# sandialabs/PyNucleus

Hardware: AMD Instinct MI355X
Metric: element-pairs/sec assembled (2D P1 fractional s=0.5, dense) + % fp64 roofline (higher is better)
Workload: dtype f64; 1 GPU; 2D unit disc (uniform_disc refined 7x, 98304 cells), P1, 48769 DoFs, fractional s=0.5, horizon=inf, dense getDense incl. zeroExterior; 4831887360 element pairs/step; noRef=7, num_dofs=48769, num_cells=98304, parallelism=block rows of the upper triangle dealt over 1 GPU(s), row-owned one-sided slabs

## Files before the change

include/pnl_hip.h:

```cpp
#ifndef PNL_HIP_H
#define PNL_HIP_H
#include <stdint.h>

#ifdef __cplusplus
extern "C" {
#endif

typedef struct pnl_context pnl_context;

enum pnl_status {
    PNL_OK = 0,
    PNL_ERR_INVALID = -1,
    PNL_ERR_UNSUPPORTED = -2,
    PNL_ERR_HIP = -3,
    PNL_ERR_STATE = -4,
    PNL_ERR_ORDER = -5
};

enum pnl_kernel_type { PNL_FRACTIONAL = 0, PNL_INDICATOR = 1, PNL_PERIDYNAMIC = 2, PNL_GAUSSIAN = 3, PNL_EXPONENTIAL = 4,
                       PNL_GAUSSIAN_BOUNDARY = 5, PNL_EXPONENTIAL_BOUNDARY = 6 };

typedef struct {
    int32_t ktype;
    int32_t interaction;
// ... 133 lines not shown

int pnl_set_order_function(pnl_context *ctx, const pnl_order_function *f, const double *cell_smax, const double *facet_smax,
                           double c0, double bc0, double sing_fac, double bsing_fac);
int pnl_set_order_vertex_values(pnl_context *ctx, int nv, const double *values_host);
int pnl_upload_pointwise_rules(pnl_context *ctx, int which, int panel, int nkeys, int M, int rows, const double *nodes,
                               const double *w, const double *phi0, const double *phi1);
int pnl_assemble_dense_pointwise(pnl_context *ctx, double *A, int64_t ldA, int zero_exterior, int cell_begin, int cell_end,
                                 int npairs, const int32_t *pairs, int nbpairs, const int32_t *bpairs);
int pnl_assemble_pairs_masked_pointwise(pnl_context *ctx, int np, const int32_t *pairs, const uint64_t *masks, const int32_t *rule,
                                        double *data);
int pnl_assemble_boundary_masked_pointwise(pnl_context *ctx, int ni, const int32_t *cells, const int32_t *facets, const uint32_t *masks,
                                           const int32_t *rule, const double *sv, double fac, double *data, double *diag);

int pnl_get_counters(pnl_context *ctx, int64_t *out, int n);
int pnl_get_phase_ms(pnl_context *ctx, float *out, int n);
int pnl_get_settled_tiles(pnl_context *ctx, int32_t *tiles, int64_t ntiles);
int pnl_get_settled_lists(pnl_context *ctx, uint16_t *codes, uint16_t *lists, int64_t ntiles);
int pnl_uniform_lane_layout(int nc, const int32_t *cells, const int32_t *dofs, int mode, int nthreads, int32_t *sizes, uint8_t *lane_cell,
                            int16_t *lds_col, int8_t *vorder, int16_t *cell_col, double *mult, double *seconds);
enum pnl_kernel_slot { PNL_K_TILE_GENERAL = 0, PNL_K_TILE_UNIFORM2, PNL_K_TILE_UNIFORM3, PNL_K_TILE_UNIFORM4, PNL_K_FOLD_MIRROR,
                       PNL_K_WORKLIST, PNL_K_TILE_SETTLED, PNL_NUM_KERNEL_SLOTS };
int pnl_get_kernel_ms(pnl_context *ctx, float *out, int n);

typedef struct pnl_tree pnl_tree;
typedef struct pnl_nfplan pnl_nfplan;
int pnl_tree_build(int N, int dim, const double *boxes, const int64_t *d2c_ptr, const int32_t *d2c_idx, int nc, double eta,
                   int min_size, int max_levels, int do_admissibility, pnl_tree **out);
int pnl_tree_build_blocks(int N, int dim, const double *boxes, const int64_t *d2c_ptr, const int32_t *d2c_idx, int nc, double eta,
                          int min_size, int max_levels, int do_admissibility, const int32_t *dof_block, int mixed_block,
                          pnl_tree **out);
// ... 174 lines not shown
```

pynucleus_amd/_lib.py:

```python
import ctypes as C
import os
import numpy as np

_HERE = os.path.dirname(os.path.abspath(__file__))
LIB_PATH = os.environ.get('PNL_LIB', os.path.join(_HERE, 'libpnl_hip.so'))

PNL_OK = 0
PNL_ERR_INVALID = -1
PNL_ERR_UNSUPPORTED = -2
PNL_ERR_HIP = -3
PNL_ERR_STATE = -4
PNL_ERR_ORDER = -5
PNL_INTERIOR = 0
PNL_BOUNDARY = 1
PNL_FLAG_NO_MIRROR = 1
PNL_FLAG_SYMMETRIC_FLUSH = 2
PNL_NUM_COUNTERS = 140

EXPORTS = ['pnl_create', 'pnl_destroy', 'pnl_error_string', 'pnl_version', 'pnl_set_stream', 'pnl_synchronize',
           'pnl_upload_mesh', 'pnl_upload_dofmap', 'pnl_set_kernel', 'pnl_set_order_formula', 'pnl_upload_distant_rules',
           'pnl_upload_singular_rule', 'pnl_upload_boundary', 'pnl_assemble_dense', 'pnl_dense_overwrites', 'pnl_block_row_costs', 'pnl_tile_cells',
           'pnl_assemble_dense_tiles', 'pnl_get_counters', 'pnl_get_phase_ms', 'pnl_get_kernel_ms', 'pnl_get_settled_tiles', 'pnl_tree_build', 'pnl_tree_build_blocks', 'pnl_tree_build_refined', 'pnl_tree_build_horizon', 'pnl_tree_build_device', 'pnl_tree_destroy', 'pnl_tree_sizes', 'pnl_tree_get', 'pnl_tree_node_cells', 'pnl_h2_transfer_matrices', 'pnl_nfplan_build', 'pnl_nfplan_destroy', 'pnl_nfplan_sizes', 'pnl_nfplan_get', 'pnl_horizon_pattern', 'pnl_near_pattern', 'pnl_pattern_set_max_nnz', 'pnl_set_option', 'pnl_set_cell_order', 'pnl_set_interaction_transform', 'pnl_set_order_vertex_values', 'pnl_h2_get', 'pnl_h2_set', 'pnl_pattern_nnz', 'pnl_pattern_get', 'pnl_pattern_destroy', 'pnl_set_row_slab', 'pnl_diag_blocks_size', 'pnl_get_diag_blocks', 'pnl_slab_matvec', 'pnl_slab_diagonal', 'pnl_gemv', 'pnl_cg_jacobi',
           'pnl_inv_diagonal', 'pnl_set_classes', 'pnl_select_class', 'pnl_upload_sparsity', 'pnl_upload_sparsity_device', 'pnl_assemble_pairs_masked', 'pnl_assemble_boundary_masked', 'pnl_assemble_clusters_tiled', 'pnl_h2_setup', 'pnl_h2_matvec', 'pnl_h2_upward', 'pnl_h2_interact', 'pnl_h2_downward', 'pnl_h2_sizes', 'pnl_spmv',
           'pnl_assemble_pairs_in_horizon', 'pnl_assemble_pairs_in_horizon_range', 'pnl_set_nonsymmetric', 'pnl_set_order_function', 'pnl_upload_pointwise_rules', 'pnl_assemble_dense_pointwise',
           'pnl_assemble_pairs_masked_pointwise', 'pnl_assemble_boundary_masked_pointwise', 'pnl_get_settled_lists',
           'pnl_gemv_axpby', 'pnl_csr_matvec', 'pnl_mg_create', 'pnl_mg_destroy', 'pnl_mg_cycle', 'pnl_mg_solve', 'pnl_mg_cg', 'pnl_theta_step', 'pnl_selftest',
           'pnl_potrf', 'pnl_potrs', 'pnl_getrf', 'pnl_getrs',
           'pnl_csr_cg_jacobi', 'pnl_fe_space_create', 'pnl_fe_space_destroy', 'pnl_assemble_nonlinearity', 'pnl_imex_create',
           'pnl_imex_destroy', 'pnl_imex_sweep', 'pnl_lincomb', 'pnl_gemv_multi', 'pnl_gemv_block', 'pnl_spmv_block', 'pnl_uniform_lane_layout',
           'pnl_h2_matvec_block', 'pnl_h2_upward_block', 'pnl_h2_interact_block', 'pnl_h2_downward_block',
           'pnl_cg_jacobi_block', 'pnl_cgb_init', 'pnl_cgb_update', 'pnl_cgb_refresh', 'pnl_cgb_direction',
           'pnl_cgb_residual', 'pnl_cgb_start', 'pnl_cgb_step', 'pnl_cgb_beta', 'pnl_mg_cycle_block', 'pnl_mg_cg_block',
           'pnl_bicgstab_block', 'pnl_bcgb_init', 'pnl_bcgb_start', 'pnl_bcgb_alpha', 'pnl_bcgb_omega', 'pnl_bcgb_direction']

PNL_FUN_BRUSSELATOR, PNL_FUN_CUBIC = 0, 1
PNL_IMEX_CG_MG, PNL_IMEX_CHOL = 0, 1
PNL_IMEX_MAX_STAGES, PNL_IMEX_MAX_COMP = 4, 2
PNL_INTERP_MAX_OPS = 21
PNL_CGB_MAXVEC, PNL_CGB_STATE = 16, 8
PNL_BCGB_STATE = 12
# ... 94 lines not shown
    L.pnl_selftest.argtypes = [i32, i32, i32, i32, vp, i32, vp, vp]
    L.pnl_set_order_formula.argtypes = [vp, i32, C.POINTER(pnl_order_formula)]
    L.pnl_upload_distant_rules.argtypes = [vp, i32, vp, vp, vp, vp, vp, vp, vp]
    L.pnl_upload_singular_rule.argtypes = [vp, i32, i32, i32, i32, vp, vp, vp, dbl]
    L.pnl_upload_boundary.argtypes = [vp, i32, vp]
    L.pnl_assemble_dense.argtypes = [vp, vp, i64, i32, i32, i32, i32]
    L.pnl_dense_overwrites.argtypes = [vp, i32, i32, i32]
    L.pnl_block_row_costs.argtypes = [vp, vp, i32]
    L.pnl_tile_cells.argtypes = [vp]
    L.pnl_assemble_dense_tiles.argtypes = [vp, vp, i64, i32, i32, vp, i32, i32, i32]
    L.pnl_get_counters.argtypes = [vp, vp, i32]
    L.pnl_get_phase_ms.argtypes = [vp, vp, i32]
    L.pnl_get_kernel_ms.argtypes = [vp, vp, i32]
    L.pnl_get_settled_tiles.argtypes = [vp, vp, C.c_int64]
    L.pnl_get_settled_lists.argtypes = [vp, vp, vp, C.c_int64]
    L.pnl_uniform_lane_layout.argtypes = [i32, vp, vp, i32, i32, vp, vp, vp, vp, vp, vp, vp]
    L.pnl_set_row_slab.argtypes = [vp, i32, vp, i32, vp]
    L.pnl_tree_build.argtypes = [i32, i32, vp, vp, vp, i32, dbl, i32, i32, i32, C.POINTER(vp)]
    L.pnl_tree_build_blocks.argtypes = [i32, i32, vp, vp, vp, i32, dbl, i32, i32, i32, vp, i32, C.POINTER(vp)]
    L.pnl_tree_build_refined.argtypes = [i32, i32, vp, vp, vp, i32, dbl, i32, i32, i32, vp, i32, i32, C.POINTER(vp)]
    L.pnl_tree_build_horizon.argtypes = [i32, i32, vp, vp, vp, i32, dbl, i32, i32, i32, vp, i32, i32, dbl, C.POINTER(vp)]
    L.pnl_tree_build_device.argtypes = [i32, i32, vp, vp, vp, i32, dbl, i32, i32, i32, i32, C.POINTER(vp)]
    L.pnl_tree_destroy.argtypes = [vp]
    L.pnl_tree_destroy.restype = None
    L.pnl_tree_sizes.argtypes = [vp, vp]
    L.pnl_tree_get.argtypes = [vp, vp, vp, vp, vp, vp, vp, vp, vp]
    L.pnl_tree_node_cells.argtypes = [vp, i32, vp, vp, vp]
    L.pnl_h2_transfer_matrices.argtypes = [i32, i32, i32, vp, vp, vp]
    L.pnl_nfplan_build.argtypes = [i32, i32, vp, i32, vp, i32, i32, vp, i32, vp, vp, vp, vp, i32, vp, i32, i32, C.POINTER(vp)]
    L.pnl_nfplan_destroy.argtypes = [vp]
# ... 457 lines not shown
        if n:
            self.check(min(self.L.pnl_get_settled_tiles(self.h, tiles.ctypes.data, n), 0))
        return tiles

    def settled_lists(self):
        n = self.settled_tiles().shape[0]
        codes = np.zeros((n, 512), dtype=np.uint16)
        have = self.L.pnl_get_settled_lists(self.h, codes.ctypes.data if n else None, None, n)
        self.check(min(have, 0))
        if not have:
            return codes, None
        lists = np.zeros((n, 4104), dtype=np.uint16)
        self.check(min(self.L.pnl_get_settled_lists(self.h, None, lists.ctypes.data, n), 0))
        return codes, lists

    def gemv(self, A_ptr, ldA, n, x_ptr, y_ptr, symmetric_half=False):
        self.check(self.L.pnl_gemv(self.h, C.c_void_p(A_ptr), int(ldA), int(n), C.c_void_p(x_ptr), C.c_void_p(y_ptr),
                                   int(symmetric_half)))

    def cg_jacobi(self, A_ptr, ldA, n, b_ptr, x_ptr, tol, maxiter):
        it, res = C.c_int(0), C.c_double(0.)
        self.check(self.L.pnl_cg_jacobi(self.h, C.c_void_p(A_ptr), int(ldA), int(n), C.c_void_p(b_ptr), C.c_void_p(x_ptr),
                                        float(tol), int(maxiter), C.byref(it), C.byref(res)))
        return it.value, res.value

    def gemv_axpby(self, A_ptr, ldA, nrows, ncols, x_ptr, alpha, beta, b_ptr, y_ptr):
        self.check(self.L.pnl_gemv_axpby(self.h, C.c_void_p(A_ptr), int(ldA), int(nrows), int(ncols), C.c_void_p(x_ptr), float(alpha),
                                         float(beta), C.c_void_p(b_ptr) if b_ptr else None, C.c_void_p(y_ptr)))

    @staticmethod
# ... 205 lines not shown
```

pynucleus_amd/csrc/pnl_context.h:

```cpp
#pragma once
#include <hip/hip_runtime.h>
#include <algorithm>
#include <cmath>
#include <cstdarg>
#include <cstdio>
#include <cstring>
#include <string>
#include <vector>
#include "pnl_hip.h"
#include "pnl_device.h"

constexpr int TILE_P1 = 64;
constexpr int TILE_P2 = 32;

struct DevBuf {
    void *p = nullptr;
    size_t bytes = 0;
    ~DevBuf() { release(); }
    void release() { if (p) { (void)hipFree(p); p = nullptr; bytes = 0; } }
};

enum PhaseEvent {
    EV_START = 0,
    EV_WORKLIST_DONE = 1,
// ... 1 lines not shown
    EV_SINGULAR_DONE = 3,
    EV_BOUNDARY_DONE = 4,
    EV_END = 5,
    EV_TILES_DONE = 6,
    EV_TILES_UNIFORM_DONE = 7,
    EV_COUNT = 8
};

struct AssemblyRun {
    bool ev_valid = false;
    bool tiles_launched = false, pure_launched = false;
    bool symflush = false;
    bool tile_cell_filter = true;
    bool full_tile_list = false;
    bool slot_used = false, fold_event_set = false;
    int settled_run = 0;
    int lists_run = 0;
    int tile_off = 0, n_mixed = 0, n_pure = 0;
    int wl_slots = 0;
    int uni_ctr_next = 0, uni_ctr_fresh = 0;
    int kev_n[PNL_NUM_KERNEL_SLOTS] = {}; bool kev_open[PNL_NUM_KERNEL_SLOTS] = {};
    unsigned long long visited_pairs = 0;
    bool visited_is_assembled = false;
};

struct UniLaneTables {
    std::vector<unsigned char> lane_cell;
    std::vector<short> lds_col, cell_col;
    std::vector<double> mult;
    int stride = 0;
// ... 34 lines not shown
    int orient = 0;
    std::vector<int32_t> cell_labels, facet_labels, cls_of;
    bool have_mesh = false, have_dofs = false, have_rules = false, have_boundary = false;
    bool dirty = true;
    DevProblem P;
    DevBuf b_cellv, b_ccen, b_cvol, b_ch, b_clog, b_cvid, b_cdof, b_cslot, b_blk_ndof, b_blk_dofs, b_perm, b_off, b_bary, b_w, b_phi,
        b_foff, b_fbary, b_fw, b_bvid, b_bv, b_bgeo, b_counters, b_D, b_tiles,
        b_vec[6], b_clabel, b_blabel, b_clsof, b_scal, b_wl, b_wlcount, b_tilectr, b_ttn, b_ttoff, b_tttab, b_ttwphi, b_wlsorted, b_wlaux,
        b_vertices, b_sp_indptr, b_sp_indices, b_mp_pairs, b_mp_masks, b_mp_wl, b_mp_sorted, b_mp_aux, b_bi_cells, b_bi_facets,
        b_bi_masks, b_cp[28], b_cpD, b_wlds, b_wlpair, b_h2[27];
    DevBuf b_kcls, b_fcls, b_uni, b_tilecls, b_ttwphif;
    DevBuf b_scolbase, b_srowoff, b_cpoff, b_cpslot, b_cprow, b_foldtab, b_bkcls, b_bfcls, b_bdefer, b_multitiles, b_slotA, b_candtiles, b_candq;
    int slot_S = 0, n_multitiles = 0;
    DevBuf b_codes, b_lists;
    int n_settled = 0, settled_want = -1, lists_want = -1;
    std::vector<int2> settled_tiles;
    long long code_builds = 0;
    DevBuf b_unictr;
    static constexpr int UNI_CTRS = 64;
    long long slot_total = 0;
    DevBuf b_rowmap, b_rowdof, b_colmap, b_coldof;
    DevBuf b_cholinfo;
    DevBuf b_luwork, b_lutmp;
    DevBuf b_blk_part, b_blk_xt;
    DevBuf b_kb_part;
    DevBuf b_cgb_work, b_bcgb_work;
    std::vector<int32_t> slab_rowdofs, slab_coldofs;
    int slab_rows = 0, slab_cols = 0;
    std::vector<DevKernel> kcls_host;
    std::vector<DevKernel> bkcls_host;
// ... 231 lines not shown

int pnl_pw_prepare(pnl_context *ctx, int need_boundary);
int pnl_pw_h2_interp(pnl_context *ctx);

int pnl_launch_gemv_symmetric(pnl_context *ctx, const double *A, long long ldA, int n, const double *x, double alpha, double beta,
                              const double *b, double *y);
int pnl_launch_slab_two_sided(pnl_context *ctx, const double *slab, long long ld, int nrows, int ncols, const int *rowdof, const int *coldof,
                              const double *x, double *y);

int pnl2_launch_uniform(pnl_context *ctx, int kt, const DevProblem &Pt, const int2 *tiles, const int *tile_cls, int ntiles, int q,
                        double *A, int64_t ldA, double *Dglob, const SlotOut &SO);
int pnl2_launch_p2(pnl_context *ctx, int kt, const int2 *tiles, const int *tile_cls, int ntiles, double *A, int64_t ldA,
                   int cell_begin, int cell_end, unsigned wl_cap_each, const SlotOut &SO);
int pnl2_zero_slot_tiles(pnl_context *ctx, const SlotOut &SO);
int pnl2_fold_mirror(pnl_context *ctx, const SlotOut &SO, double *A, int64_t ldA);
inline SlotOut slot_out(const pnl_context *ctx) {
    SlotOut SO;
    SO.A2 = (double*)ctx->b_slotA.p; SO.rowoff = (const long long*)ctx->b_srowoff.p; SO.colbase = (const int*)ctx->b_scolbase.p;
    SO.S = ctx->slot_S; SO.nU = ctx->nU;
    return SO;
}
```

pynucleus_amd/csrc/pnl_hip.hip:

```cpp
#include "pnl_context.h"
#include "pnl_kernels.h"
#include "pnl_bndtile.h"
#include "pnl_launch.h"

namespace {

__global__ void __launch_bounds__(PNL_NTHREADS)
k_mirror(double *__restrict__ A, long long ldA, int N) {
    __shared__ double t1[32][33], t2[32][33];
    const int nb = (N+31)/32;
    int bid = blockIdx.x;
    int bi = 0;
    {
        double fb = ((2.*nb+1.)-sqrt((2.*nb+1.)*(2.*nb+1.)-8.*bid))*0.5;
        bi = (int)fb;
        while (bi > 0 && (long long)bi*nb-(long long)bi*(bi-1)/2 > bid) bi--;
        while ((long long)(bi+1)*nb-(long long)(bi+1)*bi/2 <= bid) bi++;
    }
    const int bj = bi+(bid-(int)((long long)bi*nb-(long long)bi*(bi-1)/2));
    const int tx = threadIdx.x & 31, ty = threadIdx.x >> 5;
    for (int r = ty; r < 32; r += 8) {
        const int I = bi*32+r, J = bj*32+tx;
        t1[r][tx] = (I < N && J < N) ? A[(long long)I*ldA+J] : 0.;
        const int I2 = bj*32+r, J2 = bi*32+tx;
// ... 177 lines not shown
        if (DIM == 2 && DPE == 3) {
            int off = ctx->run.tile_off+ctx->run.n_mixed+ctx->run.n_pure;
            for (int q = 3; q <= 4; q++) {
                const int n = ctx->cls_n_uni[q-2][ctx->cur];
                if ((rc = pnl2_launch_uniform(ctx, KT, tile_problem(ctx), (const int2*)ctx->b_tiles.p+off, nullptr, n, q, A, ldA,
                                              (double*)(ctx->have_tile_order ? ctx->b_Dt.p : ctx->b_D.p), SO))) return rc;
                ctx->run.pure_launched = ctx->run.pure_launched || n > 0;
                off += n;
            }
        }
        HIPCHK(ctx, hipEventRecord(ctx->ev[EV_TILES_UNIFORM_DONE], ctx->stream));
    }
    unsigned *wlc = (unsigned*)ctx->b_wlcount.p+wl_slot;
    if (int rc = launch_mixed_tiles<DIM, DPE, TILE, KT>(ctx, wlc, A, ldA, cell_begin, cell_end, SO)) return rc;
    HIPCHK(ctx, hipEventRecord(ctx->ev[EV_TILES_DONE], ctx->stream));
    if (SO.A2) {
        if (int rc = pnl2_fold_mirror(ctx, SO, A, ldA)) return rc;
        HIPCHK(ctx, hipEventRecord(ctx->ev_fold, ctx->stream));
        ctx->run.fold_event_set = true;
    }
    return run_worklist<DIM, DPE, KT>(ctx, (const int4*)ctx->b_wl.p, wlc, ctx->wl_cap_each, A, ldA, ctx->run.symflush || SO.A2 != nullptr);
}

template <int DIM, int DPE, int KT>
int launch_singular(pnl_context *ctx, double *A, int64_t ldA, int cell_begin, int cell_end) {
    for (int s = 0; s < DIM+1; s++) {
        const int np = ctx->orient ? ctx->C().n_spairs1[s] : ctx->C().n_spairs[s];
        if (!np) continue;
        if (!ctx->C().have_sing[0][s]) return fail(ctx, PNL_ERR_STATE, "singular rule for %d common vertices not uploaded", s+1);
        const int wpb = PNL_SING_THREADS/64;
        int rc = with_slot<DIM>(s, [&](auto slot) {
            constexpr int SLOT = decltype(slot)::value;
            const int2 *pairs = (const int2*)(ctx->orient ? ctx->C().b_spairs1[SLOT].p : ctx->C().b_spairs[SLOT].p);
            return launch_singular_pairs<DIM, DPE, SLOT, KT, false>(ctx, (np+wpb-1)/wpb, pairs, np, A, ldA, cell_begin, cell_end, SparseOut{},
                                                                    nullptr, nullptr, ClusterTiles{});
        });
// ... 221 lines not shown
    const int norient = ctx->nonsym ? 2 : 1;
    if (ntiles > 0) {
        const bool single = DIM == 2 && DPE == 6;
        if (ncls*norient > PNL_WL_SLOTS) return fail(ctx, PNL_ERR_UNSUPPORTED, "more than %d order classes x orientations", PNL_WL_SLOTS);
        if ((rc = ensure(ctx, ctx->b_wlcount, sizeof(unsigned)*PNL_WL_SLOTS))) return rc;
        HIPCHK(ctx, hipMemsetAsync(ctx->b_wlcount.p, 0, sizeof(unsigned)*PNL_WL_SLOTS, ctx->stream));
        if ((rc = ensure_worklist(ctx, (double)ntiles*TILE*TILE, single ? ncls : 1))) return rc;
        ctx->run.wl_slots = single ? ncls : ncls*norient;
        if constexpr (DIM == 2 && DPE == 6) {
            const bool slot_ok = slot_eligible(ctx, ctx->run.full_tile_list, cell_begin, cell_end, flags);
            if ((rc = launch_tiles_single<DIM, DPE>(ctx, A, ldA, ctx->run.tile_cell_filter ? cell_begin : 0, ctx->run.tile_cell_filter ? cell_end : ctx->nc, slot_ok)))
                return rc;
        } else {
        SlotOut SO{};
        if (slot_eligible(ctx, ctx->run.full_tile_list, cell_begin, cell_end, flags) && slot_storage_ready(ctx)) { SO = slot_out(ctx); ctx->run.slot_used = true; }
        ClassScope cls(ctx, 0);
        for (int ko = 0; ko < ncls*norient; ko++) {
            const int k = ko/norient;
            cls.select(k, ko%norient);
            ctx->run.tile_off = ctx->cls_tile_off[k]; ctx->run.n_mixed = ctx->cls_n_mixed[k]; ctx->run.n_pure = ctx->cls_n_pure[k];
            if (ctx->run.n_mixed+ctx->run.n_pure+ctx->cls_n_uni[1][k]+ctx->cls_n_uni[2][k] == 0) continue;
            const int tb0 = ctx->run.tile_cell_filter ? cell_begin : 0, tb1 = ctx->run.tile_cell_filter ? cell_end : ctx->nc;
            if (ctx->P.k.fast && ctx->P.k.qm == 6 && DPE == 3) rc = launch_tiles<DIM, DPE, TILE, (DPE == 3 ? 2 : 1)>(ctx, ko, A, ldA, tb0, tb1, SO);
            else rc = with_kt(ctx->P.k.fast, [&](auto kt) { return launch_tiles<DIM, DPE, TILE, decltype(kt)::value>(ctx, ko, A, ldA, tb0, tb1, SO); });
            if (rc) return rc;
        }
        }
    }
    HIPCHK(ctx, hipEventRecord(ctx->ev[EV_WORKLIST_DONE], ctx->stream));
    if (!ctx->run.slot_used && !(flags & (PNL_FLAG_NO_MIRROR | PNL_FLAG_SYMMETRIC_FLUSH))) {
        const long long nb = (ctx->N+31)/32;
        hipLaunchKernelGGL(k_mirror, dim3((unsigned)(nb*(nb+1)/2)), dim3(PNL_NTHREADS), 0, ctx->stream, A, (long long)ldA, ctx->N);
        HIPCHK(ctx, hipGetLastError());
    }
    HIPCHK(ctx, hipEventRecord(ctx->ev[EV_MIRROR_DONE], ctx->stream));
    hipStream_t const main_stream = ctx->stream;
    bool fold_like = ctx->run.fold_event_set;
    if (!fold_like && ncls*norient == 1 && zero_exterior && !pnl_tune("PNL_NO_OVERLAP")) {
        HIPCHK(ctx, hipEventRecord(ctx->ev_fold, ctx->stream));
        fold_like = true;
    }
    const bool overlap = fold_like && ncls*norient == 1 && !pnl_tune("PNL_NO_OVERLAP");
    hipEvent_t const chain = (ctx->run.fold_event_set && !overlap && !pnl_tune("PNL_NO_OVERLAP")) ? ctx->ev_fold : nullptr;
    if (overlap) HIPCHK(ctx, hipStreamWaitEvent(ctx->aux[0], ctx->ev_fold, 0));
    {
        StreamScope on(ctx, overlap ? ctx->aux[0] : main_stream);
        ClassScope cls(ctx, 0);
        ClassFork fork(ctx, ncls*norient, chain);
        if (norient == 1 && ncls > pnl_context::NAUX && (int)ctx->cls_n_mixed.size() == ncls) fork.plan(ctx->cls_n_mixed);
        for (int ko = 0; ko < ncls*norient; ko++) {
            cls.select(ko/norient, ko%norient);
            fork.use(ko);
            rc = with_kt(ctx->P.k.fast, [&](auto kt) { return launch_singular<DIM, DPE, decltype(kt)::value>(ctx, A, ldA, cell_begin, cell_end); });
            if (rc) return rc;
        }
    }
    if (overlap) HIPCHK(ctx, hipEventRecord(ctx->ev_join[0], ctx->aux[0]));
    else HIPCHK(ctx, hipEventRecord(ctx->ev[EV_SINGULAR_DONE], ctx->stream));
    if (zero_exterior) {
        if (ctx->run.fold_event_set) rc = boundary_side(ctx->ev[EV_TILES_DONE]);
        else if (overlap) rc = boundary_side(ctx->ev_fold);
        else rc = boundary_term(chain);
        if (rc) return rc;
    }
    if (overlap) {
        HIPCHK(ctx, hipStreamWaitEvent(main_stream, ctx->ev_join[0], 0));
        HIPCHK(ctx, hipEventRecord(ctx->ev[EV_SINGULAR_DONE], ctx->stream));
    }
    if (bnd_side) HIPCHK(ctx, hipStreamWaitEvent(main_stream, ctx->ev_join[1], 0));
    HIPCHK(ctx, hipEventRecord(ctx->ev[EV_BOUNDARY_DONE], ctx->stream));
    if (ctx->slab_rows == 0) {
        scatter_diag<DPE>(ctx, ctx->P, (const double*)ctx->b_D.p, A, ldA);
        if (ctx->have_tile_order) scatter_diag<DPE>(ctx, tile_problem(ctx), (const double*)ctx->b_Dt.p, A, ldA);
// ... 496 lines not shown
```

pynucleus_amd/csrc/pnl_setup.hip:

```cpp
#include <hip/hip_runtime.h>
#include <algorithm>
#include <chrono>
#include <cmath>
#include <cstdio>
#include <cstring>
#include <deque>
#include <map>
#include <mutex>
#include <string>
#include <thread>
#include <vector>
#include "pnl_hip.h"
#include "pnl_context.h"

template <class F>
static void host_threads(F body, int want = 0) {
    const int nthr = want > 0 ? std::min(want, 64) : (int)std::max(1u, std::min(8u, std::thread::hardware_concurrency()));
    std::vector<std::thread> pool;
    for (int th = 0; th < nthr; th++) pool.emplace_back([&body, th, nthr]() { body(th, nthr); });
    for (auto &t : pool) t.join();
}

struct TileOrderJob {
    std::vector<int> cells, lperm;
// ... 784 lines not shown
    "PNL_FH_NOTILES",
    "PNL_NO_POWTAB",
    "PNL_VERBOSE",
    "PNL_PLAN_TIMING",
    "PNL_PLAN_THREADS",
    "PNL_BND_OLD",
    "PNL_NO_OVERLAP",
    "PNL_NO_FORK",
    "PNL_TILE_WGS",
    "PNL_UNI_GENERIC",
    "PNL_UNI_CHECKED",
    "PNL_UNI_LANES",
    "PNL_MIXED_GENERIC",
    "PNL_MIXED_UNSETTLED",
    "PNL_SETTLED_CODES",
};
}

const char *pnl_tune(const char *name) {
    {
        std::lock_guard<std::mutex> lk(g_opt_mutex);
        auto it = g_options.find(name);
        if (it != g_options.end()) return it->second->c_str();
    }
    return nullptr;
}

extern "C" {

const char *pnl_version(void) {
// ... 477 lines not shown
    std::vector<int> stat(cand.size());
    if ((rc = pnl_tile_pair_codes(ctx, to_dev(R.forms[0]), (const int2*)ctx->b_candtiles.p, (int)cand.size(), nullptr, stat.data()))) return rc;
    std::vector<size_t> keep;
    for (size_t c = 0; c < cand.size(); c++) if (stat[c] >= 0) keep.push_back(c);
    if (keep.empty()) return PNL_OK;
    if (ensure(ctx, ctx->b_codes, keep.size()*512*sizeof(unsigned short)) != PNL_OK) {
        (void)hipGetLastError();
        ctx->err.clear();
        return PNL_OK;
    }
    std::stable_sort(keep.begin(), keep.end(), [&](size_t x, size_t y) { return stat[x] > stat[y]; });
    for (size_t c : keep) { settled.push_back(cand[c]); is_settled[open_234[c]] = 1; }
    return PNL_OK;
}

static void tile_lists_per_class(pnl_context *ctx, const TilePlan &R, std::vector<int2> &all) {
    const std::vector<std::vector<int2>> &mixed = R.mixed, *uni = R.uni;
    for (int k = 0; k < R.ncls; k++) {
        ctx->cls_tile_off[k] = (int)all.size(); ctx->cls_n_mixed[k] = (int)mixed[k].size();
        all.insert(all.end(), mixed[k].begin(), mixed[k].end());
        for (int u = 0; u < 3; u++) { ctx->cls_n_uni[u][k] = (int)uni[u][k].size(); all.insert(all.end(), uni[u][k].begin(), uni[u][k].end()); }
        ctx->cls_n_pure[k] = ctx->cls_n_uni[0][k];
    }
}

static int tile_lists_single_launch(pnl_context *ctx, const TilePlan &R, const std::vector<int2> &tiles, std::vector<int2> &all) {
    const int ncls = R.ncls;
    const std::vector<std::vector<int2>> &mixed = R.mixed, *uni = R.uni;
    std::vector<int32_t> allcls;
    const int norient = ctx->nonsym ? 2 : 1;
// ... 70 lines not shown
            std::sort(v.begin(), v.end());
            v.erase(std::unique(v.begin(), v.end()), v.end());
        }
    }
    ctx->cls_tile_off.assign(ncls, 0); ctx->cls_n_mixed.assign(ncls, 0); ctx->cls_n_pure.assign(ncls, 0);
    for (int u = 0; u < 3; u++) ctx->cls_n_uni[u].assign(ncls, 0);
    std::vector<std::vector<int2>> &mixed = R.mixed, *uni = R.uni;
    mixed.resize(ncls);
    for (int u = 0; u < 3; u++) uni[u].resize(ncls);
    std::vector<signed char> qof(tiles.size());
    std::vector<size_t> open_234;
    std::vector<int2> settled;
    std::vector<char> is_settled;
    int rc;
    ctx->n_settled = 0;
    for (int k = 0; k < ncls; k++) {
        if ((rc = tile_orders(ctx, R, tiles, k, qof, open_234))) return rc;
        if ((rc = settle_tiles(ctx, R, tiles, open_234, settled, is_settled))) return rc;
        for (size_t i = 0; i < tiles.size(); i++) {
            const int q = qof[i];
            if (q < 0 || is_settled[i]) continue;
            (q ? uni[q-2][k] : mixed[k]).push_back(tiles[i]);
        }
        mixed[k].insert(mixed[k].end(), settled.begin(), settled.end());
    }
    if (settled.empty()) ctx->b_codes.release();
    if (settled.empty() || !lists_wanted(ctx)) ctx->b_lists.release();
    ctx->settled_tiles.clear();
    std::vector<int2> all;
    ctx->single_launch = R.p2;
// ... 10 lines not shown
        const int first = ctx->cls_tile_off[0]+ctx->cls_n_mixed[0]-(int)settled.size();
        if ((rc = pnl_tile_pair_codes(ctx, to_dev(R.forms[0]), (const int2*)ctx->b_tiles.p+first, (int)settled.size(),
                                      (unsigned short*)ctx->b_codes.p, nullptr))) return rc;
        ctx->n_settled = (int)settled.size();
        ctx->settled_tiles = settled;
        ctx->code_builds++;
        if (lists_wanted(ctx)) {
            if (ensure(ctx, ctx->b_lists, settled.size()*PNL_LIST_STRIDE*sizeof(unsigned short)) != PNL_OK) {
                (void)hipGetLastError();
                ctx->err.clear();
                ctx->b_lists.release();
            } else if ((rc = pnl_tile_pair_lists(ctx, (const unsigned short*)ctx->b_codes.p, (int)settled.size(), (unsigned short*)ctx->b_lists.p)))
                return rc;
        }
    }
    ctx->settled_want = settled_wanted();
    ctx->lists_want = lists_wanted(ctx);
    ctx->tiles_cached = tiles; ctx->tiles_cb = cell_begin; ctx->tiles_ce = cell_end; ctx->tiles_forms = R.forms;
    ctx->tiles_filter = ctx->run.tile_cell_filter;
    return PNL_OK;
}

int pnl_make_tiles(pnl_context *ctx, std::vector<int2> &tiles, int cell_begin, int cell_end) {
    const int T = ctx->tile, nbk = ctx->nblocks;
    const int a0 = cell_begin/T, a1 = (cell_end+T-1)/T;
    for (int d = 0; d < nbk; d++)
        for (int a = a0; a < a1 && a+d < nbk; a++) tiles.push_back(make_int2(a, a+d));
    return PNL_OK;
}

// ... 185 lines not shown
}

int pnl_get_settled_lists(pnl_context *ctx, uint16_t *codes, uint16_t *lists, int64_t ntiles) {
    if (!ctx || ntiles < 0) return PNL_ERR_INVALID;
    if (!ctx->b_tiles.p || ctx->cls_n_mixed.empty()) return fail(ctx, PNL_ERR_STATE, "no tile plan yet");
    const int64_t n = std::min<int64_t>(ntiles, ctx->n_settled);
    HIPCHK(ctx, hipStreamSynchronize(ctx->stream));
    if (codes && n > 0) HIPCHK(ctx, hipMemcpy(codes, ctx->b_codes.p, (size_t)n*512*sizeof(uint16_t), hipMemcpyDeviceToHost));
    if (lists && n > 0) {
        if (!ctx->b_lists.p) return fail(ctx, PNL_ERR_STATE, "the resident tile plan keeps no pair lists");
        HIPCHK(ctx, hipMemcpy(lists, ctx->b_lists.p, (size_t)n*PNL_LIST_STRIDE*sizeof(uint16_t), hipMemcpyDeviceToHost));
    }
    return ctx->b_lists.p ? ctx->n_settled : 0;
}

int pnl_uniform_lane_layout(int nc, const int32_t *cells, const int32_t *dofs, int mode, int nthreads, int32_t *sizes, uint8_t *lane_cell,
                            int16_t *lds_col, int8_t *vorder, int16_t *cell_col, double *mult, double *seconds) {
    if (nc <= 0 || !cells || !dofs || !sizes || mode < 0 || mode > 2) return PNL_ERR_INVALID;
    const int T = 64, nblocks = (nc+T-1)/T, ncp = nblocks*T;
    std::vector<int16_t> cslot((size_t)3*ncp, -1);
    std::vector<std::vector<int>> lists(nblocks);
    int nU = 1;
    for (int b = 0; b < nblocks; b++) {
        auto &L = lists[b];
        for (int c = b*T; c < std::min(nc, (b+1)*T); c++) for (int k = 0; k < 3; k++) if (dofs[(size_t)c*3+k] >= 0) L.push_back(dofs[(size_t)c*3+k]);
        std::sort(L.begin(), L.end());
        L.erase(std::unique(L.begin(), L.end()), L.end());
        nU = std::max<int>(nU, (int)L.size());
    }
    sizes[0] = nblocks; sizes[1] = nU; sizes[2] = mode == 0 ? 0 : 16*uni_lane_cap(nU)+16; sizes[3] = ncp;
// ... 42 lines not shown
```

pynucleus_amd/csrc/pnl_tile2.h:

```cpp
#pragma once
#include "pnl_common.h"

__host__ __device__ constexpr int uni_rule_size(int dpe, int np) { return 3*np+np+np*dpe+(dpe*(dpe+1)/2)*np; }


template <bool NT>
__global__ void __launch_bounds__(256)
k_fold_mirror(const double *__restrict__ A2, const FoldEntry *__restrict__ tab, const int *__restrict__ cpoff, const int2 *__restrict__ cp,
              const long long *__restrict__ cprow, double *__restrict__ A, long long ldA, int N) {
    __shared__ double t1[32][33], t2[32][33];
    __shared__ FoldEntry s_tab[2][PNL_FOLD_TAB+1];
    const unsigned nb = (unsigned)(N+31)/32;
    const unsigned nbs = (nb+7)/8;
    const unsigned sbid = blockIdx.x >> 6, inner = blockIdx.x & 63;
    unsigned I;
    {
        const float t = 2.f*(float)nbs+1.f;
        const float fb = (t-sqrtf(fmaxf(t*t-8.f*(float)sbid, 0.f)))*0.5f;
        I = (unsigned)fmaxf(fb, 0.f);
        if (I >= nbs) I = nbs-1;
        while (I > 0 && I*nbs-I*(I-1)/2 > sbid) I--;
        while (I+1 < nbs && (I+1)*nbs-(I+1)*I/2 <= sbid) I++;
    }
    const unsigned J = I+(sbid-(I*nbs-I*(I-1)/2));
    const unsigned bi = 8*I+(inner >> 3), bj = 8*J+(inner & 7);
    if (bi > bj || bj >= nb) return;
    const int tid = threadIdx.x, tx = tid & 31, ty = tid >> 5;
    if (tid < 2*(PNL_FOLD_TAB+1)) {
        const int side = tid >= PNL_FOLD_TAB+1, k = tid-side*(PNL_FOLD_TAB+1);
        s_tab[side][k] = tab[(size_t)(side ? bj : bi)*(PNL_FOLD_TAB+1)+k];
    }
    for (int k = tid; k < 32*33; k += 256) { (&t1[0][0])[k] = 0.; (&t2[0][0])[k] = 0.; }
    __syncthreads();
    const int n0 = (int)s_tab[0][0].off, n1 = (int)s_tab[1][0].off;
    if (n0 <= PNL_FOLD_TAB && n1 <= PNL_FOLD_TAB) {
#pragma unroll
        for (int g = 0; g < 2; g++) {
            if (g && bi == bj) break;
            const int nr = g ? n1 : n0, nc = g ? n0 : n1;
            double *__restrict__ tf = g ? &t2[0][0] : &t1[0][0];
            const unsigned total = (unsigned)(nr*nc), inv = ((1u << 20)+(unsigned)nc-1u)/(unsigned)nc;
            for (unsigned base = 0; base < total; base += 8*256) {
// ... 24 lines not shown
                for (int ci = cpoff[I]; ci < cpoff[min(I+1, N)]; ci++) {
                    const int a = cp[ci].x;
                    const double *__restrict__ rowp = A2+cprow[ci];
                    for (int cj = j0; cj < j1; cj++) {
                        const int2 c2 = cp[cj];
                        if (c2.x >= a) s += rowp[c2.y];
                    }
                }
                t[r][tx] = s;
            }
        };
        gather((int)bi, (int)bj, t1);
        if (bi != bj) gather((int)bj, (int)bi, t2);
    }
    __syncthreads();
    for (int r = ty; r < 32; r += 8) {
        const int I = bi*32+r, J = bj*32+tx;
        if (I < N && J < N) {
            const double v = (bi != bj) ? t1[r][tx]+t2[tx][r] : ((r != tx) ? t1[r][tx]+t1[tx][r] : t1[r][tx]);
            if (NT) __builtin_nontemporal_store(v, A+(long long)I*ldA+J); else A[(long long)I*ldA+J] = v;
        }
        const int I2 = bj*32+r, J2 = bi*32+tx;
        if (bi != bj && I2 < N && J2 < N) {
            const double v = t2[r][tx]+t1[tx][r];
            if (NT) __builtin_nontemporal_store(v, A+(long long)I2*ldA+J2); else A[(long long)I2*ldA+J2] = v;
        }
    }
}

__global__ void __launch_bounds__(256)
k_zero_slot_tiles(const SlotOut SO, const int2 *__restrict__ tiles, const int *__restrict__ blk_ndof) {
    const int a = tiles[blockIdx.x].x, b = tiles[blockIdx.x].y;
    const int nA = blk_ndof[a], nBp = SO.colbase[b+1]-SO.colbase[b], W = SO.S-SO.colbase[a];
    double *__restrict__ base = SO.A2+SO.rowoff[a]+(SO.colbase[b]-SO.colbase[a]);
    for (int t = threadIdx.x; t < nA*nBp; t += 256) {
        const int r = t/nBp, c = t-r*nBp;
        base[(long long)r*W+c] = 0.;
    }
}

__host__ __device__ constexpr size_t uniform_fixed_lds(int dpe, int np, int tile, int nUe, bool dof_lists = true) {
// ... 1054 lines not shown
```

pynucleus_amd/csrc/pnl_tile2.hip:

```cpp
#include "pnl_context.h"
#include "pnl_tile2.h"

namespace {

template <int DPE, int NP, int KT, bool STRUCT = false>
int launch_uniform_t(pnl_context *ctx, const DevProblem &Pt, const int2 *tiles, const int *tile_cls, int ntiles, int q, double *A,
                     int64_t ldA, double *Dglob, const SlotOut &SO) {
    constexpr int TILE = DPE == 6 ? 32 : 64;
    const int nUe = (ctx->nU+1) & ~1;
    const size_t fixed = uniform_fixed_lds(DPE, NP, TILE, nUe, SO.A2 == nullptr);
    int acc_stride = nUe+1;
    while (acc_stride % 32 != 1) acc_stride++;
    if (fixed+sizeof(double)*(size_t)(nUe+1)*acc_stride > 80*1024) acc_stride = (nUe+1) | 1;
    UniLanes UL{};
    int lanes_mode = 0;
    if (DPE == 3) {
        int st = 0;
        const int rc = pnl_uni_lanes_ready(ctx, &UL, &lanes_mode, &st);
        if (rc) return rc;
        if (st > 0) acc_stride = st;
    }
    size_t lds = fixed+sizeof(double)*(size_t)(nUe+1)*acc_stride;
    if (lds > 160*1024)
        return fail(ctx, PNL_ERR_UNSUPPORTED, "a block of %d cells touches %d DoFs: LDS sub-block of %zu bytes exceeds 160 KiB", TILE, ctx->nU, lds);
// ... 117 lines not shown

int pnl2_zero_slot_tiles(pnl_context *ctx, const SlotOut &SO) {
    if (ctx->n_multitiles <= 0) return PNL_OK;
    hipLaunchKernelGGL(k_zero_slot_tiles, dim3(ctx->n_multitiles), dim3(256), 0, ctx->stream, SO, (const int2*)ctx->b_multitiles.p,
                       (const int*)ctx->b_blk_ndof.p);
    HIPCHK(ctx, hipGetLastError());
    return PNL_OK;
}

int pnl2_fold_mirror(pnl_context *ctx, const SlotOut &SO, double *A, int64_t ldA) {
    const long long nb = (ctx->N+31)/32, nbs = (nb+7)/8;
    if (nbs*(nbs+1)/2*64 >= (1ll << 31)) return fail(ctx, PNL_ERR_UNSUPPORTED, "fold pass: %d DoFs exceed the grid size", ctx->N);
    const unsigned grid = (unsigned)(nbs*(nbs+1)/2*64);
    kt_begin(ctx, PNL_K_FOLD_MIRROR);
    hipLaunchKernelGGL(k_fold_mirror<true>, dim3(grid), dim3(256), 0, ctx->stream, (const double*)SO.A2, (const FoldEntry*)ctx->b_foldtab.p, (const int*)ctx->b_cpoff.p,
                       (const int2*)ctx->b_cpslot.p, (const long long*)ctx->b_cprow.p, A, (long long)ldA, ctx->N);
    kt_end(ctx, PNL_K_FOLD_MIRROR);
    HIPCHK(ctx, hipGetLastError());
    return PNL_OK;
}
```

Before: 66.05 billion element-pairs/s.

## Flag fold blocks touched by near pairs to overlap fold with worklist

At setup the host builds a bitmap of 32x32 output blocks that unsettled tiles or touching/singular pairs can write to. Those blocks are zeroed before assembly. The fold-mirror kernel then adds into flagged blocks atomically and stores to the rest, so the near-pair worklist can run on a side stream while the fold runs, instead of waiting for it. The cost is an extra zeroing kernel, atomic adds in flagged blocks, and host-side bitmap construction. Order-dependent floating-point sums may also differ slightly.

```diff
diff --git a/include/pnl_hip.h b/include/pnl_hip.h
--- a/include/pnl_hip.h
+++ b/include/pnl_hip.h
@@ -171,6 +171,7 @@
 
 int pnl_get_counters(pnl_context *ctx, int64_t *out, int n);
 int pnl_get_phase_ms(pnl_context *ctx, float *out, int n);
+int pnl_get_fold_flags(pnl_context *ctx, int64_t *nblocks, int64_t *nflagged, uint32_t *bitmap, int64_t nwords);
 int pnl_get_settled_tiles(pnl_context *ctx, int32_t *tiles, int64_t ntiles);
 int pnl_get_settled_lists(pnl_context *ctx, uint16_t *codes, uint16_t *lists, int64_t ntiles);
 int pnl_uniform_lane_layout(int nc, const int32_t *cells, const int32_t *dofs, int mode, int nthreads, int32_t *sizes, uint8_t *lane_cell,
diff --git a/pynucleus_amd/_lib.py b/pynucleus_amd/_lib.py
--- a/pynucleus_amd/_lib.py
+++ b/pynucleus_amd/_lib.py
@@ -23,7 +23,7 @@
            'pnl_assemble_dense_tiles', 'pnl_get_counters', 'pnl_get_phase_ms', 'pnl_get_kernel_ms', 'pnl_get_settled_tiles', 'pnl_tree_build', 'pnl_tree_build_blocks', 'pnl_tree_build_refined', 'pnl_tree_build_horizon', 'pnl_tree_build_device', 'pnl_tree_destroy', 'pnl_tree_sizes', 'pnl_tree_get', 'pnl_tree_node_cells', 'pnl_h2_transfer_matrices', 'pnl_nfplan_build', 'pnl_nfplan_destroy', 'pnl_nfplan_sizes', 'pnl_nfplan_get', 'pnl_horizon_pattern', 'pnl_near_pattern', 'pnl_pattern_set_max_nnz', 'pnl_set_option', 'pnl_set_cell_order', 'pnl_set_interaction_transform', 'pnl_set_order_vertex_values', 'pnl_h2_get', 'pnl_h2_set', 'pnl_pattern_nnz', 'pnl_pattern_get', 'pnl_pattern_destroy', 'pnl_set_row_slab', 'pnl_diag_blocks_size', 'pnl_get_diag_blocks', 'pnl_slab_matvec', 'pnl_slab_diagonal', 'pnl_gemv', 'pnl_cg_jacobi',
            'pnl_inv_diagonal', 'pnl_set_classes', 'pnl_select_class', 'pnl_upload_sparsity', 'pnl_upload_sparsity_device', 'pnl_assemble_pairs_masked', 'pnl_assemble_boundary_masked', 'pnl_assemble_clusters_tiled', 'pnl_h2_setup', 'pnl_h2_matvec', 'pnl_h2_upward', 'pnl_h2_interact', 'pnl_h2_downward', 'pnl_h2_sizes', 'pnl_spmv',
            'pnl_assemble_pairs_in_horizon', 'pnl_assemble_pairs_in_horizon_range', 'pnl_set_nonsymmetric', 'pnl_set_order_function', 'pnl_upload_pointwise_rules', 'pnl_assemble_dense_pointwise',
-           'pnl_assemble_pairs_masked_pointwise', 'pnl_assemble_boundary_masked_pointwise', 'pnl_get_settled_lists',
+           'pnl_assemble_pairs_masked_pointwise', 'pnl_assemble_boundary_masked_pointwise', 'pnl_get_settled_lists', 'pnl_get_fold_flags',
            'pnl_gemv_axpby', 'pnl_csr_matvec', 'pnl_mg_create', 'pnl_mg_destroy', 'pnl_mg_cycle', 'pnl_mg_solve', 'pnl_mg_cg', 'pnl_theta_step', 'pnl_selftest',
            'pnl_potrf', 'pnl_potrs', 'pnl_getrf', 'pnl_getrs',
            'pnl_csr_cg_jacobi', 'pnl_fe_space_create', 'pnl_fe_space_destroy', 'pnl_assemble_nonlinearity', 'pnl_imex_create',
@@ -148,6 +148,7 @@
     L.pnl_get_kernel_ms.argtypes = [vp, vp, i32]
     L.pnl_get_settled_tiles.argtypes = [vp, vp, C.c_int64]
     L.pnl_get_settled_lists.argtypes = [vp, vp, vp, C.c_int64]
+    L.pnl_get_fold_flags.argtypes = [vp, vp, vp, vp, C.c_int64]
     L.pnl_uniform_lane_layout.argtypes = [i32, vp, vp, i32, i32, vp, vp, vp, vp, vp, vp, vp]
     L.pnl_set_row_slab.argtypes = [vp, i32, vp, i32, vp]
     L.pnl_tree_build.argtypes = [i32, i32, vp, vp, vp, i32, dbl, i32, i32, i32, C.POINTER(vp)]
@@ -635,6 +636,17 @@
         self.check(min(self.L.pnl_get_settled_lists(self.h, None, lists.ctypes.data, n), 0))
         return codes, lists
 
+    def fold_flags(self, bitmap=False):
+        nb, nf = C.c_int64(0), C.c_int64(0)
+        nw = self.L.pnl_get_fold_flags(self.h, C.byref(nb), C.byref(nf), None, 0)
+        self.check(min(nw, 0))
+        if not bitmap:
+            return nb.value, nf.value
+        words = np.zeros(nw, dtype=np.uint32)
+        if nw:
+            self.check(min(self.L.pnl_get_fold_flags(self.h, C.byref(nb), C.byref(nf), words.ctypes.data, nw), 0))
+        return nb.value, nf.value, words
+
     def gemv(self, A_ptr, ldA, n, x_ptr, y_ptr, symmetric_half=False):
         self.check(self.L.pnl_gemv(self.h, C.c_void_p(A_ptr), int(ldA), int(n), C.c_void_p(x_ptr), C.c_void_p(y_ptr),
                                    int(symmetric_half)))
diff --git a/pynucleus_amd/csrc/pnl_context.h b/pynucleus_amd/csrc/pnl_context.h
--- a/pynucleus_amd/csrc/pnl_context.h
+++ b/pynucleus_amd/csrc/pnl_context.h
@@ -39,6 +39,7 @@
     bool tile_cell_filter = true;
     bool full_tile_list = false;
     bool slot_used = false, fold_event_set = false;
+    bool fold_flags = false;
     int settled_run = 0;
     int lists_run = 0;
     int tile_off = 0, n_mixed = 0, n_pure = 0;
@@ -103,6 +104,9 @@
     int slot_S = 0, n_multitiles = 0;
     DevBuf b_codes, b_lists;
     int n_settled = 0, settled_want = -1, lists_want = -1;
+    DevBuf b_foldflags, b_foldlist;
+    std::vector<unsigned> fold_bitmap;
+    long long fold_nblocks = 0, fold_nflagged = 0;
     std::vector<int2> settled_tiles;
     long long code_builds = 0;
     DevBuf b_unictr;
@@ -364,6 +368,7 @@
                    int cell_begin, int cell_end, unsigned wl_cap_each, const SlotOut &SO);
 int pnl2_zero_slot_tiles(pnl_context *ctx, const SlotOut &SO);
 int pnl2_fold_mirror(pnl_context *ctx, const SlotOut &SO, double *A, int64_t ldA);
+int pnl2_zero_fold_blocks(pnl_context *ctx, double *A, int64_t ldA);
 inline SlotOut slot_out(const pnl_context *ctx) {
     SlotOut SO;
     SO.A2 = (double*)ctx->b_slotA.p; SO.rowoff = (const long long*)ctx->b_srowoff.p; SO.colbase = (const int*)ctx->b_scolbase.p;
diff --git a/pynucleus_amd/csrc/pnl_hip.hip b/pynucleus_amd/csrc/pnl_hip.hip
--- a/pynucleus_amd/csrc/pnl_hip.hip
+++ b/pynucleus_amd/csrc/pnl_hip.hip
@@ -215,12 +215,23 @@
     unsigned *wlc = (unsigned*)ctx->b_wlcount.p+wl_slot;
     if (int rc = launch_mixed_tiles<DIM, DPE, TILE, KT>(ctx, wlc, A, ldA, cell_begin, cell_end, SO)) return rc;
     HIPCHK(ctx, hipEventRecord(ctx->ev[EV_TILES_DONE], ctx->stream));
-    if (SO.A2) {
+    const bool near_first = ctx->run.fold_flags && pnl_tune("PNL_NEAR_FIRST");
+    if (SO.A2 && !near_first) {
         if (int rc = pnl2_fold_mirror(ctx, SO, A, ldA)) return rc;
         HIPCHK(ctx, hipEventRecord(ctx->ev_fold, ctx->stream));
         ctx->run.fold_event_set = true;
     }
-    return run_worklist<DIM, DPE, KT>(ctx, (const int4*)ctx->b_wl.p, wlc, ctx->wl_cap_each, A, ldA, ctx->run.symflush || SO.A2 != nullptr);
+    const bool sym = ctx->run.symflush || SO.A2 != nullptr;
+    if (ctx->run.fold_flags && !near_first && !pnl_tune("PNL_NO_OVERLAP")) {
+        hipStream_t const side = ctx->aux[2];
+        HIPCHK(ctx, hipStreamWaitEvent(side, ctx->ev[EV_TILES_DONE], 0));
+        const int rc = [&] { StreamScope on(ctx, side); return run_worklist<DIM, DPE, KT>(ctx, (const int4*)ctx->b_wl.p, wlc, ctx->wl_cap_each, A, ldA, sym); }();
+        if (rc) return rc;
+        HIPCHK(ctx, hipEventRecord(ctx->ev_join[2], side));
+        HIPCHK(ctx, hipStreamWaitEvent(ctx->stream, ctx->ev_join[2], 0));
+        return PNL_OK;
+    }
+    return run_worklist<DIM, DPE, KT>(ctx, (const int4*)ctx->b_wl.p, wlc, ctx->wl_cap_each, A, ldA, sym);
 }
 
 template <int DIM, int DPE, int KT>
@@ -472,6 +483,10 @@
         } else {
         SlotOut SO{};
         if (slot_eligible(ctx, ctx->run.full_tile_list, cell_begin, cell_end, flags) && slot_storage_ready(ctx)) { SO = slot_out(ctx); ctx->run.slot_used = true; }
+        if (ctx->run.slot_used && DIM == 2 && DPE == 3 && ncls*norient == 1 && ctx->fold_nblocks > 0 && !pnl_tune("PNL_FOLD_PLAIN")) {
+            ctx->run.fold_flags = true;
+            if ((rc = pnl2_zero_fold_blocks(ctx, A, ldA))) return rc;
+        }
         ClassScope cls(ctx, 0);
         for (int ko = 0; ko < ncls*norient; ko++) {
             const int k = ko/norient;
@@ -493,14 +508,15 @@
     }
     HIPCHK(ctx, hipEventRecord(ctx->ev[EV_MIRROR_DONE], ctx->stream));
     hipStream_t const main_stream = ctx->stream;
+    const bool near_first = ctx->run.fold_flags && !ctx->run.fold_event_set && pnl_tune("PNL_NEAR_FIRST");
     bool fold_like = ctx->run.fold_event_set;
-    if (!fold_like && ncls*norient == 1 && zero_exterior && !pnl_tune("PNL_NO_OVERLAP")) {
+    if (!fold_like && !near_first && ncls*norient == 1 && zero_exterior && !pnl_tune("PNL_NO_OVERLAP")) {
         HIPCHK(ctx, hipEventRecord(ctx->ev_fold, ctx->stream));
         fold_like = true;
     }
     const bool overlap = fold_like && ncls*norient == 1 && !pnl_tune("PNL_NO_OVERLAP");
     hipEvent_t const chain = (ctx->run.fold_event_set && !overlap && !pnl_tune("PNL_NO_OVERLAP")) ? ctx->ev_fold : nullptr;
-    if (overlap) HIPCHK(ctx, hipStreamWaitEvent(ctx->aux[0], ctx->ev_fold, 0));
+    if (overlap) HIPCHK(ctx, hipStreamWaitEvent(ctx->aux[0], ctx->run.fold_flags ? ctx->ev[EV_TILES_DONE] : ctx->ev_fold, 0));
     {
         StreamScope on(ctx, overlap ? ctx->aux[0] : main_stream);
         ClassScope cls(ctx, 0);
@@ -515,6 +531,7 @@
     }
     if (overlap) HIPCHK(ctx, hipEventRecord(ctx->ev_join[0], ctx->aux[0]));
     else HIPCHK(ctx, hipEventRecord(ctx->ev[EV_SINGULAR_DONE], ctx->stream));
+    if (near_first && (rc = pnl2_fold_mirror(ctx, slot_out(ctx), A, ldA))) return rc;
     if (zero_exterior) {
         if (ctx->run.fold_event_set) rc = boundary_side(ctx->ev[EV_TILES_DONE]);
         else if (overlap) rc = boundary_side(ctx->ev_fold);
diff --git a/pynucleus_amd/csrc/pnl_setup.hip b/pynucleus_amd/csrc/pnl_setup.hip
--- a/pynucleus_amd/csrc/pnl_setup.hip
+++ b/pynucleus_amd/csrc/pnl_setup.hip
@@ -822,6 +822,8 @@
     "PNL_MIXED_GENERIC",
     "PNL_MIXED_UNSETTLED",
     "PNL_SETTLED_CODES",
+    "PNL_FOLD_PLAIN",
+    "PNL_NEAR_FIRST",
 };
 }
 
@@ -1329,6 +1331,63 @@
     return PNL_OK;
 }
 
+void pnl_fold_flag_bits(int N, int nc, int dpe, int T, const int32_t *dofs, const int2 *unsettled, size_t n_unsettled,
+                        const std::vector<int2> *touching, int ntouching, std::vector<unsigned> &bitmap, std::vector<unsigned> &list) {
+    const size_t nb = ((size_t)N+31)/32;
+    const int nblocks = (nc+T-1)/T;
+    bitmap.assign((nb*nb+31)/32, 0u);
+    list.clear();
+    auto flag = [&](int r0, int r1) {
+        const size_t k = (size_t)std::min(r0, r1)*nb+(size_t)std::max(r0, r1);
+        bitmap[k >> 5] |= 1u << (k & 31);
+    };
+    std::vector<std::vector<int>> ranges(nblocks);
+    for (int b = 0; b < nblocks; b++) {
+        std::vector<int> &v = ranges[b];
+        for (int c = b*T; c < std::min(nc, (b+1)*T); c++)
+            for (int k = 0; k < dpe; k++) { const int g = dofs[(size_t)c*dpe+k]; if (g >= 0) v.push_back(g >> 5); }
+        std::sort(v.begin(), v.end());
+        v.erase(std::unique(v.begin(), v.end()), v.end());
+    }
+    for (size_t i = 0; i < n_unsettled; i++)
+        for (int ra : ranges[unsettled[i].x]) for (int rb : ranges[unsettled[i].y]) flag(ra, rb);
+    for (int s = 0; s < ntouching; s++)
+        for (const int2 &pr : touching[s]) {
+            int r[12], n = 0;
+            for (int c : {pr.x, pr.y})
+                for (int k = 0; k < dpe && n < 12; k++) { const int g = dofs[(size_t)c*dpe+k]; if (g >= 0) r[n++] = g >> 5; }
+            for (int x = 0; x < n; x++) for (int y = x; y < n; y++) flag(r[x], r[y]);
+        }
+    for (size_t bi = 0; bi < nb; bi++)
+        for (size_t bj = bi; bj < nb; bj++) {
+            const size_t k = bi*nb+bj;
+            if ((bitmap[k >> 5] >> (k & 31)) & 1u) list.push_back((unsigned)(bi << 16 | bj));
+        }
+}
+
+static int fold_flags(pnl_context *ctx, const TilePlan &R, const std::vector<int2> &mixed, size_t n_settled) {
+    ctx->fold_nblocks = ctx->fold_nflagged = 0;
+    ctx->fold_bitmap.clear();
+    const long long nb = ((long long)ctx->N+31)/32;
+    if (!(R.p1 && ctx->dim == 2 && ctx->dpe == 3 && R.T == 64) || R.ncls != 1 || R.L > 0 || ctx->nonsym || R.cell_begin > 0 ||
+        R.cell_end < ctx->nc || nb >= (1 << 16)) return PNL_OK;
+    std::vector<unsigned> list;
+    pnl_fold_flag_bits(ctx->N, ctx->nc, ctx->dpe, R.T, ctx->dofs.data(), mixed.data(), mixed.size()-n_settled, ctx->spairs_host, 3,
+                       ctx->fold_bitmap, list);
+    if (upload(ctx, ctx->b_foldflags, ctx->fold_bitmap.data(), ctx->fold_bitmap.size()) != PNL_OK ||
+        upload(ctx, ctx->b_foldlist, list.data(), list.size()) != PNL_OK) {
+        (void)hipGetLastError();
+        ctx->err.clear();
+        ctx->fold_bitmap.clear();
+        return PNL_OK;
+    }
+    ctx->fold_nblocks = nb*(nb+1)/2; ctx->fold_nflagged = (long long)list.size();
+    if (pnl_tune("PNL_VERBOSE"))
+        fprintf(stderr, "[pnl] fold flags: %lld of %lld blocks (%.2f %%) may receive near-pair adds (%zu unsettled tiles)\n", ctx->fold_nflagged,
+                ctx->fold_nblocks, 100.*(double)ctx->fold_nflagged/(double)ctx->fold_nblocks, mixed.size()-n_settled);
+    return PNL_OK;
+}
+
 static void tile_lists_per_class(pnl_context *ctx, const TilePlan &R, std::vector<int2> &all) {
     const std::vector<std::vector<int2>> &mixed = R.mixed, *uni = R.uni;
     for (int k = 0; k < R.ncls; k++) {
@@ -1429,6 +1488,7 @@
     std::vector<char> is_settled;
     int rc;
     ctx->n_settled = 0;
+    ctx->fold_nblocks = ctx->fold_nflagged = 0;
     for (int k = 0; k < ncls; k++) {
         if ((rc = tile_orders(ctx, R, tiles, k, qof, open_234))) return rc;
         if ((rc = settle_tiles(ctx, R, tiles, open_234, settled, is_settled))) return rc;
@@ -1469,6 +1529,7 @@
                 return rc;
         }
     }
+    if ((rc = fold_flags(ctx, R, mixed[0], ctx->n_settled))) return rc;
     ctx->settled_want = settled_wanted();
     ctx->lists_want = lists_wanted(ctx);
     ctx->tiles_cached = tiles; ctx->tiles_cb = cell_begin; ctx->tiles_ce = cell_end; ctx->tiles_forms = R.forms;
@@ -1684,6 +1745,15 @@
     return ctx->b_lists.p ? ctx->n_settled : 0;
 }
 
+int pnl_get_fold_flags(pnl_context *ctx, int64_t *nblocks, int64_t *nflagged, uint32_t *bitmap, int64_t nwords) {
+    if (!ctx || !nblocks || !nflagged || nwords < 0 || (nwords && !bitmap)) return PNL_ERR_INVALID;
+    if (!ctx->b_tiles.p || ctx->cls_n_mixed.empty()) return fail(ctx, PNL_ERR_STATE, "no tile plan yet");
+    *nblocks = ctx->fold_nblocks; *nflagged = ctx->fold_nflagged;
+    const int64_t have = ctx->fold_nblocks > 0 ? (int64_t)ctx->fold_bitmap.size() : 0;
+    for (int64_t i = 0; i < nwords && i < have; i++) bitmap[i] = ctx->fold_bitmap[(size_t)i];
+    return (int)std::min<int64_t>(have, 0x7fffffff);
+}
+
 int pnl_uniform_lane_layout(int nc, const int32_t *cells, const int32_t *dofs, int mode, int nthreads, int32_t *sizes, uint8_t *lane_cell,
                             int16_t *lds_col, int8_t *vorder, int16_t *cell_col, double *mult, double *seconds) {
     if (nc <= 0 || !cells || !dofs || !sizes || mode < 0 || mode > 2) return PNL_ERR_INVALID;
diff --git a/pynucleus_amd/csrc/pnl_tile2.h b/pynucleus_amd/csrc/pnl_tile2.h
--- a/pynucleus_amd/csrc/pnl_tile2.h
+++ b/pynucleus_amd/csrc/pnl_tile2.h
@@ -7,7 +7,7 @@
 template <bool NT>
 __global__ void __launch_bounds__(256)
 k_fold_mirror(const double *__restrict__ A2, const FoldEntry *__restrict__ tab, const int *__restrict__ cpoff, const int2 *__restrict__ cp,
-              const long long *__restrict__ cprow, double *__restrict__ A, long long ldA, int N) {
+              const long long *__restrict__ cprow, double *__restrict__ A, long long ldA, int N, const unsigned *__restrict__ flags) {
     __shared__ double t1[32][33], t2[32][33];
     __shared__ FoldEntry s_tab[2][PNL_FOLD_TAB+1];
     const unsigned nb = (unsigned)(N+31)/32;
@@ -26,6 +26,8 @@
     const unsigned bi = 8*I+(inner >> 3), bj = 8*J+(inner & 7);
     if (bi > bj || bj >= nb) return;
     const int tid = threadIdx.x, tx = tid & 31, ty = tid >> 5;
+    bool flagged = false;
+    if (flags) { const unsigned k = bi*nb+bj; flagged = ((flags[k >> 5] >> (k & 31)) & 1u) != 0; }
     if (tid < 2*(PNL_FOLD_TAB+1)) {
         const int side = tid >= PNL_FOLD_TAB+1, k = tid-side*(PNL_FOLD_TAB+1);
         s_tab[side][k] = tab[(size_t)(side ? bj : bi)*(PNL_FOLD_TAB+1)+k];
@@ -80,17 +82,27 @@
         if (bi != bj) gather((int)bj, (int)bi, t2);
     }
     __syncthreads();
+    auto images = [&](auto put) {
+        for (int r = ty; r < 32; r += 8) {
+            const int I = bi*32+r, J = bj*32+tx;
+            if (I < N && J < N) put(A+(long long)I*ldA+J, (bi != bj) ? t1[r][tx]+t2[tx][r] : ((r != tx) ? t1[r][tx]+t1[tx][r] : t1[r][tx]));
+            const int I2 = bj*32+r, J2 = bi*32+tx;
+            if (bi != bj && I2 < N && J2 < N) put(A+(long long)I2*ldA+J2, t2[r][tx]+t1[tx][r]);
+        }
+    };
+    if (flagged) images([](double *p, double v) { atomic_add_f64(p, v); });
+    else images([](double *p, double v) { if (NT) __builtin_nontemporal_store(v, p); else *p = v; });
+}
+
+__global__ void __launch_bounds__(256)
+k_zero_fold_blocks(const unsigned *__restrict__ list, double *__restrict__ A, long long ldA, int N) {
+    const unsigned e = list[blockIdx.x], bi = e >> 16, bj = e & 0xffffu;
+    const int tx = threadIdx.x & 31, ty = threadIdx.x >> 5;
     for (int r = ty; r < 32; r += 8) {
         const int I = bi*32+r, J = bj*32+tx;
-        if (I < N && J < N) {
-            const double v = (bi != bj) ? t1[r][tx]+t2[tx][r] : ((r != tx) ? t1[r][tx]+t1[tx][r] : t1[r][tx]);
-            if (NT) __builtin_nontemporal_store(v, A+(long long)I*ldA+J); else A[(long long)I*ldA+J] = v;
-        }
+        if (I < N && J < N) A[(long long)I*ldA+J] = 0.;
         const int I2 = bj*32+r, J2 = bi*32+tx;
-        if (bi != bj && I2 < N && J2 < N) {
-            const double v = t2[r][tx]+t1[tx][r];
-            if (NT) __builtin_nontemporal_store(v, A+(long long)I2*ldA+J2); else A[(long long)I2*ldA+J2] = v;
-        }
+        if (bi != bj && I2 < N && J2 < N) A[(long long)I2*ldA+J2] = 0.;
     }
 }
 
diff --git a/pynucleus_amd/csrc/pnl_tile2.hip b/pynucleus_amd/csrc/pnl_tile2.hip
--- a/pynucleus_amd/csrc/pnl_tile2.hip
+++ b/pynucleus_amd/csrc/pnl_tile2.hip
@@ -155,8 +155,17 @@
     const unsigned grid = (unsigned)(nbs*(nbs+1)/2*64);
     kt_begin(ctx, PNL_K_FOLD_MIRROR);
     hipLaunchKernelGGL(k_fold_mirror<true>, dim3(grid), dim3(256), 0, ctx->stream, (const double*)SO.A2, (const FoldEntry*)ctx->b_foldtab.p, (const int*)ctx->b_cpoff.p,
-                       (const int2*)ctx->b_cpslot.p, (const long long*)ctx->b_cprow.p, A, (long long)ldA, ctx->N);
+                       (const int2*)ctx->b_cpslot.p, (const long long*)ctx->b_cprow.p, A, (long long)ldA, ctx->N,
+                       ctx->run.fold_flags ? (const unsigned*)ctx->b_foldflags.p : (const unsigned*)nullptr);
     kt_end(ctx, PNL_K_FOLD_MIRROR);
     HIPCHK(ctx, hipGetLastError());
     return PNL_OK;
 }
+
+int pnl2_zero_fold_blocks(pnl_context *ctx, double *A, int64_t ldA) {
+    if (ctx->fold_nflagged <= 0) return PNL_OK;
+    hipLaunchKernelGGL(k_zero_fold_blocks, dim3((unsigned)ctx->fold_nflagged), dim3(256), 0, ctx->stream, (const unsigned*)ctx->b_foldlist.p, A,
+                       (long long)ldA, ctx->N);
+    HIPCHK(ctx, hipGetLastError());
+    return PNL_OK;
+}
```

After: 66.45 billion element-pairs/s, median of 6. About the same (+0.6%).
